# alibaba-mmai-research/CLIP-FSAR

Measured on AMD Instinct MI355X. Metric: episodes/sec (5-way 1-shot, 8 frames, ViT-B/16), higher is better.
Workload: dtype bf16; 1 GPU; BASELINE config[1]: 5-way 1-shot, 1 query/class, 8x224^2 frames, ViT-B/16, random-init CLIP weights, synthetic structured frames; frames_per_episode=80, precision=bf16, parallelism=episodes sharded over 1 rank(s); one all-gather of accuracies, launcher=single process

## Files before the change

### clip-fsar_amd/csrc/gemm_vit.hip

```cpp
#include <type_traits>
#include <utility>

#include "common.h"
#include "gemm_vit.h"

#include "gemm_vit_epi.h"

namespace {

template <typename TI, typename TO, int ACT, int MODE, int OPATH, int STORE, bool SHORTK = false, int MIW = 4>
__global__ __launch_bounds__(512, 2) void vit_gemm_kernel(VitGemmArgs p) {
    static_assert(!SHORTK || OPATH == 1, "K = 128 runs on the LDS-DMA path");
    static_assert(MIW == 4 || (MIW == 3 && !SHORTK), "tile height 256 or 192");
    constexpr int TMv = 64 * MIW;
    constexpr int WR = 32 * MIW;
    constexpr int NM = 2 * MIW;
    constexpr int NL = MIW + 2;
    constexpr bool WIDE = MODE == 6;
    constexpr bool HAS_RES = MODE == 1 || WIDE;
    constexpr bool LNFOLD = MODE == 2 || MODE == 4;
    constexpr bool HB = MODE == 4;
    extern __shared__ __attribute__((aligned(16))) char smem[];
    const int tid = threadIdx.x, lane = tid & 63;
    const int wave = __builtin_amdgcn_readfirstlane(tid >> 6);
// ... 103 lines not shown
    };
    auto tail_pin = [&]() __attribute__((always_inline)) {
        if constexpr (CORR) asm volatile("" : "+v"(tcq[0]), "+v"(tcq[1]));
        if constexpr (LNFOLD)
            asm volatile("" : "+v"(tl[0]), "+v"(tl[1]), "+v"(tl[2]), "+v"(tl[3]), "+v"(tl[4]), "+v"(tl[5]), "+v"(tl[6]), "+v"(tl[7]), "+v"(tl[8]), "+v"(tl[NTL - 1]));
        else
            asm volatile("" : "+v"(tl[0]), "+v"(tl[1]));
    };
    auto tail_fold = [&]() __attribute__((always_inline)) {
        if constexpr (!LNFOLD) {
            typedef typename Vec2B<TI>::v8 TI8;
            TI8 bw[2];
#pragma unroll
            for (int ni = 0; ni < 2; ++ni) {
                const float bv = hi ? 0.f : tl[ni];
                const TI h = (TI)bv;
                const float r1 = bv - (float)h;
                const TI m = (TI)r1;
                const TI l = (TI)(r1 - (float)m);
                TI q = (TI)0.f;
                if constexpr (CORR) q = (TI)tcq[ni];
                bw[ni] = TI8{h, m, l, q, 0, 0, 0, 0};
            }
            const TI one = (TI)(hi ? 0.f : 1.f);
            TI8 ones = TI8{one, one, one, 0, 0, 0, 0, 0};
#pragma unroll
            for (int mi = 0; mi < MIW; ++mi) {
                if constexpr (CORR) {
                    const bool in0 = mi * 32 + lr < corr_bnd;
                    const TI ind = (TI)((p.corr != nullptr && ((in0 ? corr_par : corr_par ^ 1) == hi)) ? 1.f : 0.f);
                    ones = TI8{one, one, one, ind, 0, 0, 0, 0};
                }
#pragma unroll
                for (int ni = 0; ni < 2; ++ni) {
                    if constexpr (std::is_same<TI, _Float16>::value) acc[mi][ni] = __builtin_amdgcn_mfma_f32_32x32x16_f16(bw[ni], ones, acc[mi][ni], 0, 0, 0);
                    else acc[mi][ni] = __builtin_amdgcn_mfma_f32_32x32x16_bf16(bw[ni], ones, acc[mi][ni], 0, 0, 0);
                }
            }
        } else {
            f16x8 cw[2], mx[4];
#pragma unroll
            for (int ni = 0; ni < 2; ++ni) {
                const _Float16 h = (_Float16)tl[ni], l = (_Float16)(tl[ni] - (float)h);
                _Float16 q = (_Float16)0.f;
                if constexpr (CORR) q = (_Float16)tcq[ni];
                cw[ni] = f16x8{h, h, l, q, 0, 0, 0, 0};
            }
#pragma unroll
            for (int mi = 0; mi < MIW; ++mi) {
                const float nm = hi ? tl[2 + mi] : -tl[2 + mi];
                const _Float16 h = (_Float16)nm, l = (_Float16)(nm - (float)h);
                _Float16 sdh = (_Float16)0.f;
                if constexpr (CORR) {
                    const bool in0 = mi * 32 + lr < corr_bnd;
                    sdh = (_Float16)((p.corr != nullptr && ((in0 ? corr_par : corr_par ^ 1) == hi)) ? (p.corr_raw ? 1.0f : __builtin_amdgcn_rcpf(tl[6 + mi])) : 0.f);
                }
                mx[mi] = f16x8{h, l, h, sdh, 0, 0, 0, 0};
                rscale[mi] = tl[6 + mi];
            }
#pragma unroll
            for (int mi = 0; mi < MIW; ++mi)
#pragma unroll
                for (int ni = 0; ni < 2; ++ni)
                    acc[mi][ni] = __builtin_amdgcn_mfma_f32_32x32x16_f16(cw[ni], mx[mi], acc[mi][ni], 0, 0, 0);
        }
    };
    constexpr bool kFuseStats = LNFOLD && OPATH == 2 && MIW == 3;
    const bool fuse_stats = kFuseStats && p.part != nullptr;
    u32x4 sp[4] = {};
    auto stat_loads = [&](auto MI_) __attribute__((always_inline)) {
        constexpr int mi = decltype(MI_)::value;
        int m = m0 + wm * WR + mi * 32 + lr;
        m = m < p.M ? m : p.M - 1;
        const char* src = reinterpret_cast<const char*>(p.part) + ((size_t)m * p.part_slots + (hi ? 8 : 0)) * 8;
        sp[2] = u32x4{0u, 0u, 0u, 0u};
        sp[3] = u32x4{0u, 0u, 0u, 0u};
#ifndef CFSAR_HIDDEN_TAIL_LOADS
        sp[0] = *reinterpret_cast<const u32x4*>(src);
        sp[1] = *reinterpret_cast<const u32x4*>(src + 16);
        if (p.part_slots == 16 || hi == 0) {
            sp[2] = *reinterpret_cast<const u32x4*>(src + 32);
            sp[3] = *reinterpret_cast<const u32x4*>(src + 48);
        }
#else
        asm volatile("global_load_dwordx4 %0, %1, off" : "=v"(sp[0]) : "v"(src) : "memory");
        asm volatile("global_load_dwordx4 %0, %1, off offset:16" : "=v"(sp[1]) : "v"(src) : "memory");
        if (p.part_slots == 16 || hi == 0) {
            asm volatile("global_load_dwordx4 %0, %1, off offset:32" : "+v"(sp[2]) : "v"(src) : "memory");
            asm volatile("global_load_dwordx4 %0, %1, off offset:48" : "+v"(sp[3]) : "v"(src) : "memory");
        }
#endif
    };
    auto stat_consume = [&](auto MI_) __attribute__((always_inline)) {
        constexpr int mi = decltype(MI_)::value;
        asm volatile("" : "+v"(sp[0]), "+v"(sp[1]), "+v"(sp[2]), "+v"(sp[3]));
        auto f = [](unsigned u) { return __builtin_bit_cast(float, u); };
        float s = ((f(sp[0][0]) + f(sp[0][2])) + (f(sp[1][0]) + f(sp[1][2]))) + ((f(sp[2][0]) + f(sp[2][2])) + (f(sp[3][0]) + f(sp[3][2])));
        float sq = ((f(sp[0][1]) + f(sp[0][3])) + (f(sp[1][1]) + f(sp[1][3]))) + ((f(sp[2][1]) + f(sp[2][3])) + (f(sp[3][1]) + f(sp[3][3])));
        const int partner = (lane ^ 32) << 2;
        s += __builtin_bit_cast(float, __builtin_amdgcn_ds_bpermute(partner, __builtin_bit_cast(int, s)));
        sq += __builtin_bit_cast(float, __builtin_amdgcn_ds_bpermute(partner, __builtin_bit_cast(int, sq)));
        const float invD = p.part_invD, eps = p.part_eps;
        const float mean = s * invD;
        const float var = fmaxf(sq * invD - mean * mean, 0.f);
        const float sd = sqrtf(var + eps);
        tl[2 + mi] = hi ? sd : mean;
        tl[6 + mi] = 1.0f / sd;
    };
    auto stats_at = [&](int kstat) __attribute__((always_inline)) {
        if constexpr (kFuseStats) {
            if (fuse_stats && kstat >= 0 && kstat <= MIW) {
                static_for<MIW>([&](auto MI_) {
                    if (kstat == decltype(MI_)::value + 1) stat_consume(MI_);
                });
                static_for<MIW>([&](auto MI_) {
                    if (kstat == decltype(MI_)::value) stat_loads(MI_);
                });
            }
        }
    };
    u32x4 GX[4], GW[4];
    uint4 xfA[4], wfA[2], xfB[4], wfB[2];
    auto gloadX = [&](const unsigned (&ox)[4], int kt, auto J) __attribute__((always_inline)) {
        GX[decltype(J)::value] = *reinterpret_cast<const u32x4*>(p.A + (size_t)(kt >= p.nka ? kt - p.nka : kt) * akstride + ox[decltype(J)::value]);
    };
    auto gloadW = [&](const unsigned (&ow)[4], int kt, auto J) __attribute__((always_inline)) {
        GW[decltype(J)::value] = *reinterpret_cast<const u32x4*>(p.W + (size_t)kt * ROWB + ow[decltype(J)::value]);
    };
    auto swriteX = [&](int stage, auto J) __attribute__((always_inline)) {
        *reinterpret_cast<u32x4*>(smem + stage * STAGE + wr_off + decltype(J)::value * 8192) = GX[decltype(J)::value];
    };
    auto swriteW = [&](int stage, auto J) __attribute__((always_inline)) {
        *reinterpret_cast<u32x4*>(smem + stage * STAGE + TM * ROWB + wr_off + decltype(J)::value * 8192) = GW[decltype(J)::value];
    };
    auto dmaX = [&](const unsigned (&ox)[4], int kt, int stage, auto J) __attribute__((always_inline)) {
        const char* src = p.A + (size_t)(kt >= p.nka ? kt - p.nka : kt) * akstride + ox[decltype(J)::value];
        const unsigned dst = ldsw + (unsigned)stage * (unsigned)STAGE + (unsigned)decltype(J)::value * 8192u;
#ifdef CFSAR_DEV
        if (p.dbg & 4096) { glds16_asm_pol<1>(src, dst); return; }
        if (p.dbg & 16384) { glds16_asm_pol<2>(src, dst); return; }
#endif
        glds16_asm(src, dst);
    };
    auto dmaW = [&](const unsigned (&ow)[4], int kt, int stage, auto J) __attribute__((always_inline)) {
        const char* src = p.W + (size_t)kt * ROWB + ow[decltype(J)::value];
        const unsigned dst = ldsw + (unsigned)stage * (unsigned)STAGE + (unsigned)(TM * ROWB) + (unsigned)decltype(J)::value * 8192u;
#ifdef CFSAR_DEV
        if (p.dbg & 8192) { glds16_asm_pol<1>(src, dst); return; }
#endif
        glds16_asm(src, dst);
    };
    using T_ = std::true_type;
    using F_ = std::false_type;
    auto load_one = [&](int stage, int ss, auto J, uint4 (&xf)[4], uint4 (&wf)[2]) __attribute__((always_inline)) {
        constexpr int j = decltype(J)::value;
        const char* base = smem + stage * STAGE;
        const int x2 = ss << 5;
        constexpr int isx[6] = {1, 0, 1, 1, MIW == 4 ? 1 : 0, 0};
        constexpr int idx[6] = {0, 0, 1, 2, MIW == 4 ? 3 : 1, 1};
        if constexpr (isx[j] != 0) xf[idx[j]] = *reinterpret_cast<const uint4*>(base + (rdX[idx[j]] ^ x2));
        else wf[idx[j]] = *reinterpret_cast<const uint4*>(base + (rdW[idx[j]] ^ x2));
    };
    auto mfma_one = [&](auto J, uint4 (&xf)[4], uint4 (&wf)[2], auto ZERO) __attribute__((always_inline)) {
        constexpr int j = decltype(J)::value;
        constexpr int ni = j / MIW, mi = j % MIW;
        const f32x16 zero = {0.f, 0.f, 0.f, 0.f, 0.f, 0.f, 0.f, 0.f, 0.f, 0.f, 0.f, 0.f, 0.f, 0.f, 0.f, 0.f};
        const f32x16 c = decltype(ZERO)::value ? zero : acc[mi][ni];
        if constexpr (std::is_same<TI, _Float16>::value)
            acc[mi][ni] = __builtin_amdgcn_mfma_f32_32x32x16_f16(__builtin_bit_cast(f16x8, wf[ni]), __builtin_bit_cast(f16x8, xf[mi]), c, 0, 0, 0);
        else
            acc[mi][ni] = __builtin_amdgcn_mfma_f32_32x32x16_bf16(__builtin_bit_cast(bf16x8, wf[ni]), __builtin_bit_cast(bf16x8, xf[mi]), c, 0, 0, 0);
    };
    auto step = [&](int cur, int nxt, const unsigned (&ox)[4], const unsigned (&ow)[4], int ksrc, auto LOAD, auto WRITE, auto SYNC, auto FRAGS, auto ZERO, auto TAIL, int kstat = -1) __attribute__((always_inline)) {
        constexpr bool load = decltype(LOAD)::value, write = decltype(WRITE)::value, sync = decltype(SYNC)::value,
                       frags = decltype(FRAGS)::value, tail = decltype(TAIL)::value;
        static_for<NM>([&](auto J) {
            constexpr int j = decltype(J)::value;
            mfma_one(J, xfA, wfA, ZERO);
            if constexpr (j < NL) load_one(cur, 1, J, xfB, wfB);
            if constexpr (j >= NM - MIW) {
                if constexpr (OPATH == 0) { if constexpr (write) swriteX(nxt, std::integral_constant<int, j - (NM - MIW)>{}); }
                else if constexpr (OPATH == 1) { if constexpr (load) dmaX(ox, ksrc, nxt, std::integral_constant<int, j - (NM - MIW)>{}); }
            }
            __builtin_amdgcn_sched_barrier(0);
        });
        static_for<NM>([&](auto J) {
            constexpr int j = decltype(J)::value;
            mfma_one(J, xfB, wfB, F_{});
            if constexpr (j < NL) load_one(cur, 2, J, xfA, wfA);
            if constexpr (OPATH == 0) {
                if constexpr (j >= NM - MIW && load) gloadX(ox, ksrc, std::integral_constant<int, j - (NM - MIW)>{});
            } else if constexpr (OPATH == 1) {
                if constexpr (j >= NM - 4 && load) dmaW(ow, ksrc, nxt, std::integral_constant<int, j - (NM - 4)>{});
            }
            __builtin_amdgcn_sched_barrier(0);
        });
        static_for<NM>([&](auto J) {
            constexpr int j = decltype(J)::value;
            mfma_one(J, xfA, wfA, F_{});
            if constexpr (j < NL) load_one(cur, 3, J, xfB, wfB);
            if constexpr (j >= NM - 4 && OPATH == 0 && write) swriteW(nxt, std::integral_constant<int, j - (NM - 4)>{});
            __builtin_amdgcn_sched_barrier(0);
        });
        static_for<NM>([&](auto J) {
            constexpr int j = decltype(J)::value;
            mfma_one(J, xfB, wfB, F_{});
            if constexpr (j < 2) {
                if constexpr (OPATH == 0 && load) {
                    gloadW(ow, ksrc, std::integral_constant<int, 2 * j>{});
                    gloadW(ow, ksrc, std::integral_constant<int, 2 * j + 1>{});
                }
            } else if constexpr (frags) {
                load_one(nxt, 0, std::integral_constant<int, j - 2>{}, xfA, wfA);
                if constexpr (j == NM - 1 && NL > NM - 2) load_one(nxt, 0, std::integral_constant<int, NL - 1>{}, xfA, wfA);
            }
            if constexpr (tail && j == 2) tail_loads(m0, n0);
            if constexpr (kFuseStats && j == 2) stats_at(kstat);
            if constexpr (OPATH == 2 && load && j >= 2 && MIW == 4) {
                if constexpr (j < 6) dmaX(ox, ksrc, cur, std::integral_constant<int, j - 2>{});
                else {
                    dmaW(ow, ksrc, cur, std::integral_constant<int, 2 * (j - 6)>{});
                    dmaW(ow, ksrc, cur, std::integral_constant<int, 2 * (j - 6) + 1>{});
                }
            }
            if constexpr (OPATH == 2 && load && j >= 2 && MIW == 3) {
                if constexpr (j == 2) { dmaX(ox, ksrc, cur, std::integral_constant<int, 0>{}); dmaX(ox, ksrc, cur, std::integral_constant<int, 1>{}); }
                if constexpr (j == 3) { dmaX(ox, ksrc, cur, std::integral_constant<int, 2>{}); dmaW(ow, ksrc, cur, std::integral_constant<int, 0>{}); }
                if constexpr (j == 4) { dmaW(ow, ksrc, cur, std::integral_constant<int, 1>{}); dmaW(ow, ksrc, cur, std::integral_constant<int, 2>{}); }
                if constexpr (j == 5) { dmaW(ow, ksrc, cur, std::integral_constant<int, 3>{}); }
            }
            __builtin_amdgcn_sched_barrier(0);
            if constexpr (j == 1 && sync) {
                if constexpr (OPATH >= 1) asm volatile("s_waitcnt vmcnt(0)" ::: "memory");
#ifndef CFSAR_HIDDEN_TAIL_LOADS
                if constexpr (!frags && OPATH >= 1) tail_pin();
#endif
                __syncthreads();
                __builtin_amdgcn_sched_barrier(0);
            }
        });
    };
    origin(b, m0, n0);
    unsigned offX[4], offW[4];
    offsets(m0, n0, offX, offW);
    if constexpr (OPATH == 0) {
        static_for<MIW>([&](auto J) { gloadX(offX, 0, J); });
        static_for<4>([&](auto J) { gloadW(offW, 0, J); });
        static_for<MIW>([&](auto J) { swriteX(0, J); });
        static_for<4>([&](auto J) { swriteW(0, J); });
        static_for<MIW>([&](auto J) { gloadX(offX, 1, J); });
        static_for<4>([&](auto J) { gloadW(offW, 1, J); });
    } else {
        static_for<MIW>([&](auto J) { dmaX(offX, 0, 0, J); });
        static_for<4>([&](auto J) { dmaW(offW, 0, 0, J); });
        if constexpr (OPATH == 2) {
            static_for<MIW>([&](auto J) { dmaX(offX, 1, 1, J); });
            static_for<4>([&](auto J) { dmaW(offW, 1, 1, J); });
            asm volatile("s_waitcnt vmcnt(%0)" : : "n"(MIW + 4) : "memory");
        } else {
            asm volatile("s_waitcnt vmcnt(0)" ::: "memory");
        }
    }
    __syncthreads();
#ifdef CFSAR_DEV
    if (p.dbg & 32768) {
        if (wave >= 4) __builtin_amdgcn_s_setprio(1);
    }
    if (p.dbg & 65536) {
        if (wave < 4) __builtin_amdgcn_s_setprio(1);
    }
#endif
    int sb = 0;
    char* slab = smem + EPI_OFF + wave * EPI_SLAB;
#ifdef CFSAR_DEV
    int trace_i = 0;
    if (p.dbg & 128) {
        const int n = ((blockIdx.x >> 3) & 31) * p.stagger_unit;
        for (int i = 0; i < n; ++i) __builtin_amdgcn_s_sleep(1);
        __syncthreads();
    }
#define CFSAR_TRACE(slot) do { if (p.trace && tid == 0 && trace_i < 64) p.trace[((size_t)blockIdx.x * 64 + trace_i) * 4 + (slot)] = (long long)__builtin_amdgcn_s_memrealtime(); } while (0)
#else
#define CFSAR_TRACE(slot) do { } while (0)
#endif
    for (;;) {
        const int bn = b + grid;
        const bool has_next = bn < nt;
        int m0n = m0, n0n = n0;
        if (has_next) origin(bn, m0n, n0n);
        static_for<NL>([&](auto J) { load_one(sb, 0, J, xfA, wfA); });
        CFSAR_TRACE(0);
        int kt = 0;
        u32x4 rv0[4] = {};
        auto residual_prefetch = [&]() __attribute__((always_inline)) {
            if constexpr (HAS_RES && !WIDE && OPATH >= 1) {
                const int mb_ = m0 + wm * WR, nb_ = n0 + wn * 64;
                const int ncl_ = nb_ + 64 <= p.N ? nb_ : p.N - 64;
                const int rr_ = lane >> 3, Q_ = lane & 7;
#pragma unroll
                for (int it = 0; it < 4; ++it) {
                    int row = mb_ + rr_ + it * 8;
                    row = row < p.M ? row : p.M - 1;
                    rv0[it] = *reinterpret_cast<const u32x4*>(reinterpret_cast<const char*>(p.res) + ((size_t)row * p.ldr + ncl_ + 8 * Q_) * 2);
                }
            }
        };
        if constexpr (OPATH == 0) {
            step(sb & 1, (sb + 1) & 1, offX, offW, 2, T_{}, T_{}, T_{}, T_{}, T_{}, F_{});
            for (kt = 1; kt < nk - 2; ++kt) step((sb + kt) & 1, (sb + kt + 1) & 1, offX, offW, kt + 2, T_{}, T_{}, T_{}, T_{}, F_{}, F_{});
            offsets(m0n, n0n, offX, offW);
            step((sb + kt) & 1, (sb + kt + 1) & 1, offX, offW, 0, T_{}, T_{}, T_{}, T_{}, F_{}, T_{});
            ++kt;
            step((sb + kt) & 1, (sb + kt + 1) & 1, offX, offW, 1, T_{}, T_{}, T_{}, F_{}, F_{}, F_{});
            asm volatile("s_waitcnt vmcnt(%0)" : : "n"(MIW + 4) : "memory");
        } else if constexpr (OPATH == 1 && SHORTK) {
            step(sb & 1, (sb + 1) & 1, offX, offW, 1, T_{}, F_{}, T_{}, T_{}, T_{}, T_{});
            kt = 1;
            offsets(m0n, n0n, offX, offW);
            residual_prefetch();
            step((sb + kt) & 1, (sb + kt + 1) & 1, offX, offW, 0, T_{}, F_{}, T_{}, F_{}, F_{}, F_{});
        } else if constexpr (OPATH == 1) {
            step(sb & 1, (sb + 1) & 1, offX, offW, 1, T_{}, F_{}, T_{}, T_{}, T_{}, F_{});
            for (kt = 1; kt < nk - 2; ++kt) step((sb + kt) & 1, (sb + kt + 1) & 1, offX, offW, kt + 1, T_{}, F_{}, T_{}, T_{}, F_{}, F_{});
            step((sb + kt) & 1, (sb + kt + 1) & 1, offX, offW, kt + 1, T_{}, F_{}, T_{}, T_{}, F_{}, T_{});
            ++kt;
            offsets(m0n, n0n, offX, offW);
            residual_prefetch();
            step((sb + kt) & 1, (sb + kt + 1) & 1, offX, offW, 0, T_{}, F_{}, T_{}, F_{}, F_{}, F_{});
        } else {
            step(sb & 1, (sb + 1) & 1, offX, offW, 2, T_{}, F_{}, T_{}, T_{}, T_{}, F_{}, 0);
            for (kt = 1; kt < nk - 2; ++kt) step((sb + kt) & 1, (sb + kt + 1) & 1, offX, offW, kt + 2, T_{}, F_{}, T_{}, T_{}, F_{}, F_{}, kt);
            offsets(m0n, n0n, offX, offW);
            step((sb + kt) & 1, (sb + kt + 1) & 1, offX, offW, 0, T_{}, F_{}, T_{}, T_{}, F_{}, T_{});
            ++kt;
            residual_prefetch();
            step((sb + kt) & 1, (sb + kt + 1) & 1, offX, offW, 1, T_{}, F_{}, T_{}, F_{}, F_{}, F_{});
        }
        tail_pin();
        tail_fold();
        CFSAR_TRACE(1);
#ifdef CFSAR_DEV
        if (p.dbg & 4) {
            if (acc[0][0][0] == 123.456f) reinterpret_cast<float*>(p.out)[0] = acc[1][1][3] + acc[MIW - 1][1][2] + acc[2][0][1];
        } else
#endif
        {
            const int mb = m0 + wm * WR, nb = n0 + wn * 64;
            if constexpr (WIDE) {
                if (mb + WR <= p.M && nb + 64 <= p.N) epilogue_rows_wide<STORE, true, MIW>(acc, p, mb, nb, lane, slab);
                else epilogue_rows_wide<STORE, false, MIW>(acc, p, mb, nb, lane, slab);
            } else
            if (mb + WR <= p.M && nb + 64 <= p.N) epilogue_rows<TO, ACT, HAS_RES, STORE, true, LNFOLD, HAS_RES && OPATH >= 1, HB, MIW>(acc, p, mb, nb, lane, slab, rscale, rv0);
            else epilogue_rows<TO, ACT, HAS_RES, STORE, false, LNFOLD, HAS_RES && OPATH >= 1, HB, MIW>(acc, p, mb, nb, lane, slab, rscale, rv0);
        }
        CFSAR_TRACE(2);
#ifdef CFSAR_DEV
        ++trace_i;
#endif
        if (!has_next) {
            if constexpr (OPATH == 2) asm volatile("s_waitcnt vmcnt(0)" ::: "memory");
            break;
        }
        sb = (sb + nk) & 1;
        b = bn;
        m0 = m0n;
        n0 = n0n;
    }
}

int persistent_grid() {
    const int n = cfsar_num_cus() & ~7;
    return n >= 8 ? n : 8;
}

constexpr bool vit_has_192(int mode, int opath) {
    return mode == 1 || mode == 6 || ((mode == 2 || mode == 4) && opath == 2);
}

int vit_pick_miw(int M, int tiles_n, int mode, int opath, int K, int dbg) {
    if (K == 128 || !vit_has_192(mode, opath)) return 4;
    const long long G = persistent_grid();
    const long long t256 = (long long)((M + 255) / 256) * tiles_n, t192 = (long long)((M + 191) / 192) * tiles_n;
    const long long r256 = ((t256 + G - 1) / G) * 256, r192 = ((t192 + G - 1) / G) * 192;
    int miw = r192 * 10 <= r256 * 9 ? 3 : 4;
#ifdef CFSAR_DEV
    if (dbg & (1 << 17)) miw = 3;
    if (dbg & (1 << 18)) miw = 4;
#endif
    (void)dbg;
    return miw;
}

template <typename TI, typename TO, int ACT, int MODE, int OPATH, int STORE, bool SHORTK, int MIW = 4>
int launch_inst2(const VitGemmArgs& a, hipStream_t s) {
    auto* fn = &vit_gemm_kernel<TI, TO, ACT, MODE, OPATH, STORE, SHORTK, MIW>;
    if (int rc = cfsar_ensure_lds(reinterpret_cast<const void*>(fn), LDS_BYTES, "cfsar_gemm(vit)")) return rc;
    const int grid = a.ntiles < persistent_grid() ? ((a.ntiles + 7) & ~7) : persistent_grid();
    hipLaunchKernelGGL(fn, dim3(grid), dim3(512), LDS_BYTES, s, a);
    return cfsar_check_launch("cfsar_gemm(vit)");
}

template <typename TI, typename TO, int ACT, int MODE, int OPATH, int STORE>
int launch_inst(const VitGemmArgs& a, hipStream_t s) {
    if (a.K == 128) return launch_inst2<TI, TO, ACT, MODE, 1, STORE, true>(a, s);
    if constexpr (vit_has_192(MODE, OPATH)) {
        if (a.miw == 3) return launch_inst2<TI, TO, ACT, MODE, OPATH, STORE, false, 3>(a, s);
    }
    return launch_inst2<TI, TO, ACT, MODE, OPATH, STORE, false>(a, s);
}

template <int OPATH, int STORE>
int launch_path(const VitGemmArgs& a, int mode, bool f16io, hipStream_t s) {
    if constexpr (STORE == 0) {
        if (mode == 5) return launch_inst<__bf16, __bf16, CFSAR_ACT_NONE, 1, OPATH, STORE>(a, s);
        if (mode == 6) return launch_inst<_Float16, _Float16, CFSAR_ACT_NONE, 6, OPATH, STORE>(a, s);
        if (mode == 1) {
            if (f16io) return launch_inst<_Float16, _Float16, CFSAR_ACT_NONE, 1, OPATH, STORE>(a, s);
            return launch_inst<__bf16, _Float16, CFSAR_ACT_NONE, 1, OPATH, STORE>(a, s);
        }
    } else {
        if (mode == 2) {
            if (f16io) {
                if (a.hb_tokens > 0) return -2;
                if (a.act == CFSAR_ACT_QUICKGELU) return launch_inst<_Float16, _Float16, CFSAR_ACT_QUICKGELU, 2, OPATH, STORE>(a, s);
                return launch_inst<_Float16, _Float16, CFSAR_ACT_NONE, 2, OPATH, STORE>(a, s);
            }
            if (a.act == CFSAR_ACT_QUICKGELU) return launch_inst<_Float16, __bf16, CFSAR_ACT_QUICKGELU, 2, OPATH, STORE>(a, s);
            if (a.hb_tokens > 0) return launch_inst<_Float16, __bf16, CFSAR_ACT_NONE, 4, OPATH, STORE>(a, s);
            return launch_inst<_Float16, __bf16, CFSAR_ACT_NONE, 2, OPATH, STORE>(a, s);
        }
        if (mode == 0) {
            if (a.act == CFSAR_ACT_QUICKGELU) return launch_inst<__bf16, __bf16, CFSAR_ACT_QUICKGELU, 0, OPATH, STORE>(a, s);
            if (a.relu) return launch_inst<__bf16, __bf16, kActRelu, 0, OPATH, STORE>(a, s);
            return launch_inst<__bf16, __bf16, CFSAR_ACT_NONE, 0, OPATH, STORE>(a, s);
        }
    }
    return cfsar_fail("cfsar_gemm (vit): internal: no instance of mode %d with store policy %d", mode, STORE);
}

}

#ifdef CFSAR_DEV
static int g_stagger_unit = 0;
static long long* g_trace = nullptr;
#endif
int cfsar_gemm_vit_try(const VitGemmCall& c, hipStream_t s) {
    const bool lnfold = c.rowstats != nullptr || c.part != nullptr;
    const bool f16io = lnfold ? c.out_dtype == CFSAR_F16 : c.in_dtype == CFSAR_F16;
    const bool f16res = !lnfold && c.out_dtype == CFSAR_F16 && c.res && c.res_dtype == CFSAR_F16 && c.act == CFSAR_ACT_NONE;
    const bool bf16plain = (c.out_dtype == CFSAR_BF16 || (lnfold && c.out_dtype == CFSAR_F16)) && !c.res &&
                           (c.act == CFSAR_ACT_NONE || c.act == CFSAR_ACT_QUICKGELU);
    const bool bf16res = !lnfold && c.in_dtype == CFSAR_BF16 && c.out_dtype == CFSAR_BF16 && c.res && c.res_dtype == CFSAR_BF16 &&
                         c.act == CFSAR_ACT_NONE && c.res != c.out;
    if (!lnfold && c.in_dtype == CFSAR_F16 && !f16res) return -2;
    const bool plainrelu = bf16plain && !lnfold && c.relu && c.act == CFSAR_ACT_NONE && c.out_dtype == CFSAR_BF16 && c.N >= 256;
    if (!(f16res || bf16plain || bf16res) || !c.bias || (c.relu && !(bf16res || plainrelu))) return -2;
    if (lnfold && (!bf16plain || !c.cvec)) return -2;
    if (c.stats_out && !f16res) return -2;
    if (c.K % 64 != 0 || c.K < 128 || c.N % 64 != 0 || c.ldo % 8 != 0 || (c.res && c.ldr % 8 != 0)) return -2;
    if ((size_t)c.M * c.lda * 2 >= (1ull << 32) || (size_t)c.N * c.ldw * 2 >= (1ull << 32) ||
        (size_t)c.M * c.ldo * 2 >= (1ull << 32)) return -2;
    VitGemmArgs a;
    a.A = static_cast<const char*>(c.A);
    a.W = static_cast<const char*>(c.W);
    a.out = c.out;
    a.bias = c.bias;
    a.res = c.res;
    a.rowstats = c.rowstats;
    const int ka = c.ka > 0 ? c.ka : c.K;
    if (!(ka == c.K || (((2 * ka == c.K && ka % 64 == 0) || (3 * ka == 2 * c.K && c.wide && ka % 128 == 0)) && ka >= 128 && c.ha_tokens == 0 &&
                        c.hb_tokens == 0 && c.in_dtype == CFSAR_F16)))
        return cfsar_fail("cfsar_gemm (vit): split operands need K = 2 ka (ka %% 64 == 0) or 2 K = 3 ka (ka %% 128 == 0), fp16 operands, row-major layouts (K=%d, ka=%d)", c.K, ka);
    if (c.wide && !(f16res && c.in_dtype == CFSAR_F16 && c.res == c.out && c.ldr == c.ldo && c.ha_tokens == 0))
        return cfsar_fail("cfsar_gemm_residual_wide: fp16 operands, the residual stream updated in place");
    a.nka = ka / 64;
    a.res_lo = c.wide ? c.res_lo : nullptr;
    a.corr = c.corr;
    a.corr_tokens = c.corr_tokens;
    a.corr_raw = c.corr_raw;
    a.colsum = c.colsum;
    if (c.colsum && !(lnfold && c.act == CFSAR_ACT_QUICKGELU && c.out_dtype == CFSAR_F16 && c.corr_tokens >= 128 && c.hb_tokens == 0))
        return cfsar_fail("cfsar_gemm_lnfold_hp: per-frame output means exist for the fp16 QuickGELU form with >= 128 tokens per frame");
    if (c.corr && !(c.corr_tokens >= 128 && c.in_dtype == CFSAR_F16 && c.out_dtype == CFSAR_F16 && (lnfold || c.wide) && c.hb_tokens == 0))
        return cfsar_fail("cfsar_gemm (vit): the per-frame correction needs >= 128 tokens per frame and an fp16-mode instance (tokens=%d)", c.corr_tokens);
    a.part = c.part; a.part_slots = c.part_slots; a.part_invD = 1.0f / (float)ka; a.part_eps = c.part_eps;
    if (c.part && !(c.pol.opath == 2 && ka >= 512 && (c.part_slots == 12 || c.part_slots == 16) && c.part_slots * 64 == ka))
        return cfsar_fail("cfsar_gemm_lnfold_partials: needs K = 64 slots in {768, 1024} (K=%d, slots=%d)", ka, c.part_slots);
    a.cvec = c.cvec;
    a.stats_out = c.stats_out;
    a.stats_slots = c.N / 64;
    a.M = c.M; a.N = c.N; a.K = c.K;
    a.lda = c.lda; a.ldw = c.ldw; a.ldo = c.ldo; a.ldr = c.ldr;
    a.act = c.act;
    a.relu = c.relu;
    a.tiles_n = (c.N + TN - 1) / TN;
    a.miw = vit_pick_miw(c.M, a.tiles_n, lnfold ? 2 : ((f16res || bf16res) ? (c.wide ? 6 : 1) : 0), c.pol.opath, c.K, c.dbg);
    if (c.part && a.miw != 3) return cfsar_fail("cfsar_gemm_lnfold_partials: internal: fused statistics need the 192-row instance");
    if (c.out_miw) *c.out_miw = a.miw;
    a.ntiles = ((c.M + 64 * a.miw - 1) / (64 * a.miw)) * a.tiles_n;
    a.group = c.pol.group;
    a.colfast = c.pol.colfast;
    a.hb_tokens = c.hb_tokens; a.hb_heads = c.hb_heads; a.ha_tokens = c.ha_tokens;
    if (a.hb_tokens > 0 && !(lnfold && c.act == CFSAR_ACT_NONE && a.hb_tokens >= 128 && a.hb_heads > 0 && c.N == 3 * 64 * a.hb_heads &&
// ... 218 lines not shown
```

### clip-fsar_amd/csrc/gemm_vit_epi.h

```cpp
#pragma once
#include <type_traits>
#include <utility>

#include "common.h"
#include "gemm_vit.h"

namespace {

typedef unsigned u32x4 __attribute__((ext_vector_type(4)));
typedef unsigned u32x2 __attribute__((ext_vector_type(2)));

template <typename F, int... Is>
__device__ __forceinline__ void static_for_impl(F&& f, std::integer_sequence<int, Is...>) {
    (f(std::integral_constant<int, Is>{}), ...);
}
template <int N, typename F>
__device__ __forceinline__ void static_for(F&& f) {
    static_for_impl(static_cast<F&&>(f), std::make_integer_sequence<int, N>{});
}

constexpr int kActRelu = 100;
constexpr int TM = 256, TN = 256;
constexpr int ROWB = 128;
constexpr int STAGE = (TM + TN) * ROWB;
constexpr int EPI_OFF = 2 * STAGE;
constexpr int EPI_SLAB = 32 * 128;
constexpr int LDS_BYTES = EPI_OFF + 8 * EPI_SLAB;

__device__ __forceinline__ int swz(int row) { return (row >> 1) & 7; }

__device__ __forceinline__ void glds16_asm(const char* src, unsigned lds_addr) {
    unsigned keep;
    asm volatile(
        "s_mov_b32 %0, m0\n\t"
        "s_mov_b32 m0, %2\n\t"
        "s_nop 0\n\t"
        "global_load_lds_dwordx4 %1, off\n\t"
        "s_mov_b32 m0, %0"
        : "=&s"(keep)
        : "v"(src), "s"(lds_addr)
        : "memory");
}

#ifdef CFSAR_DEV
template <int POL>
__device__ __forceinline__ void glds16_asm_pol(const char* src, unsigned lds_addr) {
    unsigned keep;
    if constexpr (POL == 1)
        asm volatile("s_mov_b32 %0, m0\n\ts_mov_b32 m0, %2\n\ts_nop 0\n\tglobal_load_lds_dwordx4 %1, off nt\n\ts_mov_b32 m0, %0" : "=&s"(keep) : "v"(src), "s"(lds_addr) : "memory");
    else
        asm volatile("s_mov_b32 %0, m0\n\ts_mov_b32 m0, %2\n\ts_nop 0\n\tglobal_load_lds_dwordx4 %1, off sc1\n\ts_mov_b32 m0, %0" : "=&s"(keep) : "v"(src), "s"(lds_addr) : "memory");
}
#endif

__device__ __forceinline__ void quick_gelu4(float (&v)[4]) {
#pragma unroll
    for (int j = 0; j < 4; ++j) {
        const float z = -1.702f * 1.4426950408889634f * v[j];
        v[j] = v[j] * __builtin_amdgcn_rcpf(1.0f + __builtin_amdgcn_exp2f(z));
    }
}

template <int CTRL>
__device__ __forceinline__ float dpp_move(float v) {
    return __builtin_bit_cast(float, __builtin_amdgcn_update_dpp(0, __builtin_bit_cast(int, v), CTRL, 0xF, 0xF, false));
}
__device__ __forceinline__ float dpp_sum8(float v) {
    v += dpp_move<0xB1>(v);
    v += dpp_move<0x4E>(v);
    v += dpp_move<0x141>(v);
    return v;
}

template <int POLICY>
__device__ __forceinline__ void store16(void* dst, u32x4 v) {
    if constexpr (POLICY == 2) {
        asm volatile("global_store_dwordx4 %0, %1, off sc1 nt\n\ts_nop 1" : : "v"(dst), "v"(v) : "memory");
    } else {
        *reinterpret_cast<u32x4*>(dst) = v;
    }
}

__device__ __forceinline__ void tile_of(int lin, int tiles_m, int tiles_n, int group, int colfast, int& tm, int& tn) {
    const int per = group * tiles_n;
    const int gid = lin / per, first = gid * group;
    const int gsz = tiles_m - first < group ? tiles_m - first : group;
    const int rem = lin - gid * per;
    if (colfast) {
        tm = first + rem / tiles_n;
        tn = rem - (rem / tiles_n) * tiles_n;
    } else {
        tm = first + rem % gsz;
        tn = rem / gsz;
    }
}

template <int HALF>
__device__ __forceinline__ float half_plus(unsigned pair, float c) {
    float r;
    if constexpr (HALF == 0) asm("v_fma_mix_f32 %0, %1, 1.0, %2 op_sel_hi:[1,0,0]" : "=v"(r) : "v"(pair), "v"(c));
    else asm("v_fma_mix_f32 %0, %1, 1.0, %2 op_sel:[1,0,0] op_sel_hi:[1,0,0]" : "=v"(r) : "v"(pair), "v"(c));
    return r;
}

template <typename TO, int ACT, bool HAS_RES, int STORE, bool FULL, bool ROWSCALE = false, bool PRE = false, bool HB = false, int NMI = 4, int CH = 1024>
__device__ __forceinline__ void epilogue_rows(f32x16 (&acc)[NMI][2], const VitGemmArgs& p, int mb, int nb, int lane, char* slab,
                                              const float (&rscale)[4], const u32x4 (&rv0)[4]) {
    typedef typename Vec2B<TO>::v4 TO4;
    typedef typename Vec2B<TO>::v8 TO8;
    const int lr = lane & 31, hi = lane >> 5;
    const int rr = lane >> 3, Q = lane & 7;
    constexpr bool COLSUM = std::is_same<TO, _Float16>::value && ACT == CFSAR_ACT_QUICKGELU && ROWSCALE && !HAS_RES && !HB;
    typedef _Float16 cs_h8 __attribute__((ext_vector_type(8)));
    unsigned cs0[8] = {0, 0, 0, 0, 0, 0, 0, 0}, cs1[8] = {0, 0, 0, 0, 0, 0, 0, 0};
    int cs_bnd = 0, cs_jb = 0, cs_jb0 = 0;
    if constexpr (COLSUM) {
        if (p.colsum != nullptr) {
            cs_bnd = (mb / p.corr_tokens + 1) * p.corr_tokens - mb;
            const int jb = (cs_bnd - rr + 7) >> 3;
            cs_jb = jb < 4 * NMI ? jb : 4 * NMI;
            cs_jb0 = __builtin_amdgcn_readfirstlane(cs_bnd >> 3);
        }
    }
    const bool colok = FULL || nb + 64 <= p.N;
    const int ncl = colok ? nb : p.N - 64;
    char* wr = CH == 1024 ? slab + lr * 128 : slab + (lr >> 3) * CH + (lr & 7) * 128;
    const int wsw = lr & 15;
    const bool swap_halves = rr & 1;
    const unsigned ostep = (unsigned)p.ldo * 16u, rstep = (unsigned)p.ldr * 16u;
    char* outp = reinterpret_cast<char*>(p.out) + ((size_t)(mb + rr) * p.ldo + ncl + 8 * Q) * 2;
    const char* resp = HAS_RES ? reinterpret_cast<const char*>(p.res) + ((size_t)(mb + rr) * p.ldr + ncl + 8 * Q) * 2 : nullptr;
    const int rd0 = rr * 128 + ((Q ^ ((rr >> 1) & 7)) << 4);
    char* hb_base = nullptr;
    size_t hb_wrap = 0;
    int hb_wrap_step = 16;
    if constexpr (HB) {
        const int row0 = mb + rr;
        const int f0 = row0 / p.hb_tokens, t0 = row0 - f0 * p.hb_tokens;
        const int blk = ncl >> 6, which = blk / p.hb_heads, h = blk - which * p.hb_heads;
        const size_t frame_bytes = (size_t)p.hb_heads * p.hb_tokens * 384;
        hb_base = reinterpret_cast<char*>(p.out) + (size_t)f0 * frame_bytes + ((size_t)h * p.hb_tokens + t0) * 384 + which * 128 + Q * 16;
        hb_wrap = frame_bytes - (size_t)p.hb_tokens * 384;
        hb_wrap_step = (p.hb_tokens - t0 + 7) >> 3;
    }
    auto out_addr = [&](int step) __attribute__((always_inline)) -> char* {
        if constexpr (HB) return hb_base + step * 3072 + (step >= hb_wrap_step ? hb_wrap : (size_t)0);
        else return outp + (size_t)step * ostep;
    };
    u32x4 rvn[4];
    auto load_res = [&](int mi_) __attribute__((always_inline)) {
        if constexpr (HAS_RES) {
#pragma unroll
            for (int it = 0; it < 4; ++it) {
                const int step = mi_ * 4 + it;
                if (FULL || mb + rr + step * 8 < p.M) rvn[it] = *reinterpret_cast<const u32x4*>(resp + (size_t)step * rstep);
                else rvn[it] = u32x4{0, 0, 0, 0};
            }
        }
    };
    if constexpr (PRE) {
#pragma unroll
        for (int it = 0; it < 4; ++it) rvn[it] = rv0[it];
    } else {
        load_res(0);
    }
    auto gelu_consts = [&](int mi, float& gk, float& gsd) __attribute__((always_inline)) {
        if constexpr (ROWSCALE && ACT == CFSAR_ACT_QUICKGELU) {
            float rs = rscale[mi];
            asm volatile("" : "+v"(rs));
            gk = -1.702f * 1.4426950408889634f * rs;
            gsd = __builtin_amdgcn_rcpf(rs);
        }
    };
    auto convert_group = [&](int mi, int q, float gk, float gsd) __attribute__((always_inline)) {
        const int ni = q >> 2, g = q & 3;
        TO4 o;
        float v[4];
        if constexpr (ROWSCALE && ACT == CFSAR_ACT_QUICKGELU) {
#pragma unroll
            for (int j = 0; j < 4; ++j) {
                const float a = acc[mi][ni][4 * g + j];
                const float e = __builtin_amdgcn_exp2f(a * gk);
                v[j] = a * __builtin_amdgcn_rcpf(__builtin_fmaf(e, gsd, gsd));
            }
        } else {
#pragma unroll
            for (int j = 0; j < 4; ++j) {
                v[j] = acc[mi][ni][4 * g + j];
                if constexpr (ROWSCALE) v[j] *= rscale[mi];
            }
            if constexpr (ACT == CFSAR_ACT_QUICKGELU) quick_gelu4(v);
            if constexpr (ACT == kActRelu) {
#pragma unroll
                for (int j = 0; j < 4; ++j) v[j] = fmaxf(v[j], 0.0f);
            }
        }
#pragma unroll
        for (int j = 0; j < 4; ++j) o[j] = (TO)v[j];
        const int slot = (2 * (ni * 4 + g) + hi) ^ wsw;
        *reinterpret_cast<TO4*>(wr + slot * 8) = o;
    };
    auto read_back = [&](u32x4 (&d)[4]) __attribute__((always_inline)) {
#pragma unroll
        for (int it = 0; it < 4; ++it)
            d[it] = *reinterpret_cast<const u32x4*>(slab + it * CH + (rd0 ^ ((it & 1) << 6)));
    };
    auto finish = [&](int mi, int it, u32x4 x, u32x4 r) __attribute__((always_inline)) {
        const bool rowok = FULL || mb + rr + (mi * 4 + it) * 8 < p.M;
        if (swap_halves) x = u32x4{x[2], x[3], x[0], x[1]};
        if constexpr (HAS_RES && std::is_same<TO, _Float16>::value) {
            typedef _Float16 h2 __attribute__((ext_vector_type(2)));
            const h2 ones = {(_Float16)1.0f, (_Float16)1.0f};
            float ps = 0.f, pq = 0.f;
            const TO8 s8 = __builtin_bit_cast(TO8, x) + __builtin_bit_cast(TO8, r);
            x = __builtin_bit_cast(u32x4, s8);
            if (p.stats_out) {
                const h2 s01 = __builtin_shufflevector(s8, s8, 0, 1), s23 = __builtin_shufflevector(s8, s8, 2, 3);
                const h2 s45 = __builtin_shufflevector(s8, s8, 4, 5), s67 = __builtin_shufflevector(s8, s8, 6, 7);
                ps = __builtin_amdgcn_fdot2(s01, ones, ps, false);
                pq = __builtin_amdgcn_fdot2(s01, s01, pq, false);
                ps = __builtin_amdgcn_fdot2(s23, ones, ps, false);
                pq = __builtin_amdgcn_fdot2(s23, s23, pq, false);
                ps = __builtin_amdgcn_fdot2(s45, ones, ps, false);
                pq = __builtin_amdgcn_fdot2(s45, s45, pq, false);
                ps = __builtin_amdgcn_fdot2(s67, ones, ps, false);
                pq = __builtin_amdgcn_fdot2(s67, s67, pq, false);
                ps = dpp_sum8(ps);
                pq = dpp_sum8(pq);
                if (Q == 0 && (FULL || (rowok && colok)))
                    *reinterpret_cast<float2*>(p.stats_out + ((size_t)(mb + rr + (mi * 4 + it) * 8) * p.stats_slots + (nb >> 6)) * 2) =
                        make_float2(ps, pq);
            }
        } else if constexpr (HAS_RES) {
            const TO8 a = __builtin_bit_cast(TO8, x), b = __builtin_bit_cast(TO8, r);
            TO8 sres;
#pragma unroll
            for (int j = 0; j < 8; ++j) {
                float t = (float)a[j] + (float)b[j];
                if (p.relu) t = fmaxf(t, 0.0f);
                sres[j] = (TO)t;
            }
            x = __builtin_bit_cast(u32x4, sres);
        }
#ifdef CFSAR_DEV
        if ((p.dbg & 16) && x[0] != 0x7fc12345u) return;
        if ((p.dbg & 32) && ((blockIdx.x >> 3) & 1) && x[0] != 0x7fc12345u) return;
#endif
        if (FULL || (rowok && colok)) store16<STORE>(out_addr(mi * 4 + it), x);
        if constexpr (COLSUM) {
            if (p.colsum != nullptr) {
                typedef _Float16 cs_h2 __attribute__((ext_vector_type(2)));
                const int j_ = mi * 4 + it;
                if (j_ == cs_jb0 || j_ == cs_jb0 + 1) {
#pragma unroll
                    for (int e = 0; e < 8; ++e) cs0[e] = (j_ == cs_jb) ? cs1[e] : cs0[e];
                }
                constexpr float kMagic = 1.5f * 2048.0f;
                const cs_h2 lim = {(_Float16)1000.0f, (_Float16)1000.0f};
#pragma unroll
                for (int k = 0; k < 4; ++k) {
                    const unsigned xw = x[k];
                    cs_h2 hv = __builtin_bit_cast(cs_h2, xw);
                    hv = __builtin_elementwise_min(__builtin_elementwise_max(hv, -lim), lim);
                    const unsigned cw = __builtin_bit_cast(unsigned, hv);
                    const unsigned b0 = __builtin_bit_cast(unsigned, half_plus<0>(cw, kMagic)), b1 = __builtin_bit_cast(unsigned, half_plus<1>(cw, kMagic));
                    cs1[2 * k] += (FULL || rowok) ? b0 : __builtin_bit_cast(unsigned, kMagic);
                    cs1[2 * k + 1] += (FULL || rowok) ? b1 : __builtin_bit_cast(unsigned, kMagic);
                }
            }
        }
    };
#pragma unroll
    for (int mi = 0; mi < NMI; ++mi) {
        u32x4 rv[4];
#pragma unroll
        for (int it = 0; it < 4; ++it) {
            if constexpr (HAS_RES) rv[it] = rvn[it];
        }
        if (mi < NMI - 1) load_res(mi + 1);
        float gk = 0.f, gsd = 0.f;
        gelu_consts(mi, gk, gsd);
#pragma unroll
        for (int q = 0; q < 8; ++q) convert_group(mi, q, gk, gsd);
        u32x4 d[4];
        read_back(d);
#pragma unroll
        for (int it = 0; it < 4; ++it) finish(mi, it, d[it], rv[it]);
    }
    if constexpr (COLSUM) {
        if (p.colsum != nullptr) {
            const int partner = (lane ^ 32) << 2;
            constexpr unsigned kbits = 0x45400000u;
            static_assert(__builtin_bit_cast(unsigned, 1.5f * 2048.0f) == kbits, "magic constant");
#pragma unroll
            for (int j = 0; j < 8; ++j) {
                int a0 = (int)((cs_jb >= 4 * NMI ? cs1[j] : cs0[j]) - (unsigned)cs_jb * kbits);
                int a1 = (int)(cs1[j] - (unsigned)(4 * NMI) * kbits) - a0;
                a0 += __builtin_amdgcn_update_dpp(0, a0, 0x128, 0xF, 0xF, false);
                a1 += __builtin_amdgcn_update_dpp(0, a1, 0x128, 0xF, 0xF, false);
                a0 += __builtin_amdgcn_ds_swizzle(a0, 0x401F);
                a1 += __builtin_amdgcn_ds_swizzle(a1, 0x401F);
                a0 += __builtin_amdgcn_ds_bpermute(partner, a0);
                a1 += __builtin_amdgcn_ds_bpermute(partner, a1);
                cs0[j] = (unsigned)a0;
                cs1[j] = (unsigned)a1;
            }
            if (rr == 0 && colok && mb < p.M) {
                int* dst = reinterpret_cast<int*>(p.colsum) + ((size_t)(mb / (32 * NMI)) * 2) * p.N + ncl + 8 * Q;
                *reinterpret_cast<u32x4*>(dst) = u32x4{cs0[0], cs0[1], cs0[2], cs0[3]};
                *reinterpret_cast<u32x4*>(dst + 4) = u32x4{cs0[4], cs0[5], cs0[6], cs0[7]};
                *reinterpret_cast<u32x4*>(dst + p.N) = u32x4{cs1[0], cs1[1], cs1[2], cs1[3]};
                *reinterpret_cast<u32x4*>(dst + p.N + 4) = u32x4{cs1[4], cs1[5], cs1[6], cs1[7]};
            }
        }
    }
}

template <int HALF>
__device__ __forceinline__ float mix_sum(unsigned a, unsigned b) {
    float r;
    if constexpr (HALF == 0) asm("v_fma_mix_f32 %0, %1, 1.0, %2 op_sel_hi:[1,0,1]" : "=v"(r) : "v"(a), "v"(b));
    else asm("v_fma_mix_f32 %0, %1, 1.0, %2 op_sel:[1,0,1] op_sel_hi:[1,0,1]" : "=v"(r) : "v"(a), "v"(b));
    return r;
}
template <int HALF>
__device__ __forceinline__ float mix_sub(unsigned pair, float c) {
    float r;
    if constexpr (HALF == 0) asm("v_fma_mix_f32 %0, %1, -1.0, %2 op_sel_hi:[1,0,0]" : "=v"(r) : "v"(pair), "v"(c));
    else asm("v_fma_mix_f32 %0, %1, -1.0, %2 op_sel:[1,0,0] op_sel_hi:[1,0,0]" : "=v"(r) : "v"(pair), "v"(c));
    return r;
}

template <int STORE, bool FULL, int NMI, int CH = 1024>
__device__ __forceinline__ void epilogue_rows_wide(f32x16 (&acc)[NMI][2], const VitGemmArgs& p, int mb, int nb, int lane, char* slab) {
    typedef _Float16 h2 __attribute__((ext_vector_type(2)));
    typedef _Float16 h8 __attribute__((ext_vector_type(8)));
    typedef float f4 __attribute__((ext_vector_type(4)));
    const int lr = lane & 31, hi = lane >> 5;
    const int rr = lane >> 2, Q = lane & 3;
    const bool colok = FULL || nb + 64 <= p.N;
    const int ncl = colok ? nb : p.N - 64;
    const int wsw = ((lr >> 1) & 7) ^ ((lr & 1) << 2);
    const int rsw = ((rr >> 1) & 7) ^ ((rr & 1) << 2);
    char* wr = CH == 1024 ? slab + lr * 128 : slab + (lr >> 3) * CH + (lr & 7) * 128;
    const char* rd = CH == 1024 ? slab + rr * 128 : slab + (rr >> 3) * CH + (rr & 7) * 128;
    const bool has_lo = p.res_lo != nullptr;
    const size_t eoff = ((size_t)(mb + rr) * p.ldo + ncl + 8 * Q) * 2;
    char* outp = reinterpret_cast<char*>(p.out) + eoff;
    char* lop = has_lo ? reinterpret_cast<char*>(p.res_lo) + eoff : nullptr;
    const unsigned rstep = (unsigned)p.ldo * 32u;
    u32x4 rh[2], rl[2], nh[2], nl[2];
    auto load_res = [&](int pass) __attribute__((always_inline)) {
        const int mi_ = pass >> 1, ni_ = pass & 1;
#pragma unroll
        for (int it = 0; it < 2; ++it) {
            const int step = mi_ * 2 + it;
            const bool ok = FULL || mb + rr + step * 16 < p.M;
            const size_t o = (size_t)step * rstep + ni_ * 64;
            nh[it] = ok ? *reinterpret_cast<const u32x4*>(outp + o) : u32x4{0, 0, 0, 0};
            nl[it] = (ok && has_lo) ? *reinterpret_cast<const u32x4*>(lop + o) : u32x4{0, 0, 0, 0};
        }
    };
    load_res(0);
    float ps[2] = {0.f, 0.f}, pq[2] = {0.f, 0.f};
#pragma unroll
    for (int pass = 0; pass < 2 * NMI; ++pass) {
        const int mi = pass >> 1, ni = pass & 1;
#pragma unroll
        for (int it = 0; it < 2; ++it) { rh[it] = nh[it]; rl[it] = nl[it]; }
        if (pass + 1 < 2 * NMI) load_res(pass + 1);
#pragma unroll
        for (int g = 0; g < 4; ++g) {
            const f4 v = {acc[mi][ni][4 * g], acc[mi][ni][4 * g + 1], acc[mi][ni][4 * g + 2], acc[mi][ni][4 * g + 3]};
            *reinterpret_cast<f4*>(wr + (((2 * g + hi) ^ wsw) << 4)) = v;
        }
#pragma unroll
        for (int it = 0; it < 2; ++it) {
            const f4 a = *reinterpret_cast<const f4*>(rd + it * 2 * CH + (((2 * Q) ^ rsw) << 4));
            const f4 b = *reinterpret_cast<const f4*>(rd + it * 2 * CH + (((2 * Q + 1) ^ rsw) << 4));
            u32x4 ohw, olw;
#pragma unroll
            for (int k = 0; k < 4; ++k) {
                const float d0 = k < 2 ? a[2 * k] : b[2 * k - 4], d1 = k < 2 ? a[2 * k + 1] : b[2 * k - 3];
                const float s0 = d0 + mix_sum<0>(rh[it][k], rl[it][k]);
                const float s1 = d1 + mix_sum<1>(rh[it][k], rl[it][k]);
                const h2 hp = {(_Float16)s0, (_Float16)s1};
                const unsigned hb = __builtin_bit_cast(unsigned, hp);
                const h2 lp = {(_Float16)mix_sub<0>(hb, s0), (_Float16)mix_sub<1>(hb, s1)};
                ohw[k] = hb;
                olw[k] = __builtin_bit_cast(unsigned, lp);
            }
            const h8 oh = __builtin_bit_cast(h8, ohw), ol = __builtin_bit_cast(h8, olw);
            const int step = mi * 2 + it;
            const bool rowok = FULL || mb + rr + step * 16 < p.M;
            if (p.stats_out) {
                const h2 ones = {(_Float16)1.0f, (_Float16)1.0f};
                const h2 s01 = __builtin_shufflevector(oh, oh, 0, 1), s23 = __builtin_shufflevector(oh, oh, 2, 3);
                const h2 s45 = __builtin_shufflevector(oh, oh, 4, 5), s67 = __builtin_shufflevector(oh, oh, 6, 7);
                float s_ = 0.f, q_ = 0.f;
                s_ = __builtin_amdgcn_fdot2(s01, ones, s_, false);
                q_ = __builtin_amdgcn_fdot2(s01, s01, q_, false);
                s_ = __builtin_amdgcn_fdot2(s23, ones, s_, false);
                q_ = __builtin_amdgcn_fdot2(s23, s23, q_, false);
                s_ = __builtin_amdgcn_fdot2(s45, ones, s_, false);
                q_ = __builtin_amdgcn_fdot2(s45, s45, q_, false);
                s_ = __builtin_amdgcn_fdot2(s67, ones, s_, false);
                q_ = __builtin_amdgcn_fdot2(s67, s67, q_, false);
                s_ += dpp_move<0xB1>(s_);
                q_ += dpp_move<0xB1>(q_);
                s_ += dpp_move<0x4E>(s_);
                q_ += dpp_move<0x4E>(q_);
                if (ni == 0) { ps[it] = s_; pq[it] = q_; }
                else {
                    ps[it] += s_; pq[it] += q_;
                    if (Q == 0 && (FULL || (rowok && colok)))
                        *reinterpret_cast<float2*>(p.stats_out + ((size_t)(mb + rr + step * 16) * p.stats_slots + (nb >> 6)) * 2) =
                            make_float2(ps[it], pq[it]);
                }
            }
            if (FULL || (rowok && colok)) {
                const size_t o = (size_t)step * rstep + ni * 64;
                store16<STORE>(outp + o, __builtin_bit_cast(u32x4, oh));
                if (has_lo) store16<STORE>(lop + o, __builtin_bit_cast(u32x4, ol));
            }
        }
    }
}

}
```

Before: 347.4 episodes/s.

## Overlap next tile's first k-step MFMAs with LN-fold GEMM epilogue

```diff
diff --git a/clip-fsar_amd/csrc/gemm_vit.hip b/clip-fsar_amd/csrc/gemm_vit.hip
--- a/clip-fsar_amd/csrc/gemm_vit.hip
+++ b/clip-fsar_amd/csrc/gemm_vit.hip
@@ -279,20 +279,23 @@
     };
     using T_ = std::true_type;
     using F_ = std::false_type;
-    auto load_one = [&](int stage, int ss, auto J, uint4 (&xf)[4], uint4 (&wf)[2]) __attribute__((always_inline)) {
+    auto load_one = [&](int stage, int ss, auto J, uint4 (&xf)[4], uint4 (&wf)[2], auto ONLY_LAST) __attribute__((always_inline)) {
         constexpr int j = decltype(J)::value;
         const char* base = smem + stage * STAGE;
         const int x2 = ss << 5;
         constexpr int isx[6] = {1, 0, 1, 1, MIW == 4 ? 1 : 0, 0};
         constexpr int idx[6] = {0, 0, 1, 2, MIW == 4 ? 3 : 1, 1};
-        if constexpr (isx[j] != 0) xf[idx[j]] = *reinterpret_cast<const uint4*>(base + (rdX[idx[j]] ^ x2));
-        else wf[idx[j]] = *reinterpret_cast<const uint4*>(base + (rdW[idx[j]] ^ x2));
+        if constexpr (isx[j] != 0) {
+            if constexpr (!decltype(ONLY_LAST)::value || idx[j] == MIW - 1) xf[idx[j]] = *reinterpret_cast<const uint4*>(base + (rdX[idx[j]] ^ x2));
+        } else wf[idx[j]] = *reinterpret_cast<const uint4*>(base + (rdW[idx[j]] ^ x2));
     };
     auto mfma_one = [&](auto J, uint4 (&xf)[4], uint4 (&wf)[2], auto ZERO) __attribute__((always_inline)) {
         constexpr int j = decltype(J)::value;
         constexpr int ni = j / MIW, mi = j % MIW;
+        constexpr int zmode = (int)decltype(ZERO)::value;
+        if constexpr ((zmode & 2) != 0 && mi != MIW - 1) return;
         const f32x16 zero = {0.f, 0.f, 0.f, 0.f, 0.f, 0.f, 0.f, 0.f, 0.f, 0.f, 0.f, 0.f, 0.f, 0.f, 0.f, 0.f};
-        const f32x16 c = decltype(ZERO)::value ? zero : acc[mi][ni];
+        const f32x16 c = (zmode & 1) ? zero : acc[mi][ni];
         if constexpr (std::is_same<TI, _Float16>::value)
             acc[mi][ni] = __builtin_amdgcn_mfma_f32_32x32x16_f16(__builtin_bit_cast(f16x8, wf[ni]), __builtin_bit_cast(f16x8, xf[mi]), c, 0, 0, 0);
         else
@@ -301,10 +304,12 @@
     auto step = [&](int cur, int nxt, const unsigned (&ox)[4], const unsigned (&ow)[4], int ksrc, auto LOAD, auto WRITE, auto SYNC, auto FRAGS, auto ZERO, auto TAIL, int kstat = -1) __attribute__((always_inline)) {
         constexpr bool load = decltype(LOAD)::value, write = decltype(WRITE)::value, sync = decltype(SYNC)::value,
                        frags = decltype(FRAGS)::value, tail = decltype(TAIL)::value;
+        using REST_ = std::integral_constant<int, (int)decltype(ZERO)::value & 2>;
+        using OL_ = std::integral_constant<bool, ((int)decltype(ZERO)::value & 2) != 0>;
         static_for<NM>([&](auto J) {
             constexpr int j = decltype(J)::value;
             mfma_one(J, xfA, wfA, ZERO);
-            if constexpr (j < NL) load_one(cur, 1, J, xfB, wfB);
+            if constexpr (j < NL) load_one(cur, 1, J, xfB, wfB, OL_{});
             if constexpr (j >= NM - MIW) {
                 if constexpr (OPATH == 0) { if constexpr (write) swriteX(nxt, std::integral_constant<int, j - (NM - MIW)>{}); }
                 else if constexpr (OPATH == 1) { if constexpr (load) dmaX(ox, ksrc, nxt, std::integral_constant<int, j - (NM - MIW)>{}); }
@@ -313,8 +318,8 @@
         });
         static_for<NM>([&](auto J) {
             constexpr int j = decltype(J)::value;
-            mfma_one(J, xfB, wfB, F_{});
-            if constexpr (j < NL) load_one(cur, 2, J, xfA, wfA);
+            mfma_one(J, xfB, wfB, REST_{});
+            if constexpr (j < NL) load_one(cur, 2, J, xfA, wfA, OL_{});
             if constexpr (OPATH == 0) {
                 if constexpr (j >= NM - MIW && load) gloadX(ox, ksrc, std::integral_constant<int, j - (NM - MIW)>{});
             } else if constexpr (OPATH == 1) {
@@ -324,22 +329,22 @@
         });
         static_for<NM>([&](auto J) {
             constexpr int j = decltype(J)::value;
-            mfma_one(J, xfA, wfA, F_{});
-            if constexpr (j < NL) load_one(cur, 3, J, xfB, wfB);
+            mfma_one(J, xfA, wfA, REST_{});
+            if constexpr (j < NL) load_one(cur, 3, J, xfB, wfB, OL_{});
             if constexpr (j >= NM - 4 && OPATH == 0 && write) swriteW(nxt, std::integral_constant<int, j - (NM - 4)>{});
             __builtin_amdgcn_sched_barrier(0);
         });
         static_for<NM>([&](auto J) {
             constexpr int j = decltype(J)::value;
-            mfma_one(J, xfB, wfB, F_{});
+            mfma_one(J, xfB, wfB, REST_{});
             if constexpr (j < 2) {
                 if constexpr (OPATH == 0 && load) {
                     gloadW(ow, ksrc, std::integral_constant<int, 2 * j>{});
                     gloadW(ow, ksrc, std::integral_constant<int, 2 * j + 1>{});
                 }
             } else if constexpr (frags) {
-                load_one(nxt, 0, std::integral_constant<int, j - 2>{}, xfA, wfA);
-                if constexpr (j == NM - 1 && NL > NM - 2) load_one(nxt, 0, std::integral_constant<int, NL - 1>{}, xfA, wfA);
+                load_one(nxt, 0, std::integral_constant<int, j - 2>{}, xfA, wfA, F_{});
+                if constexpr (j == NM - 1 && NL > NM - 2) load_one(nxt, 0, std::integral_constant<int, NL - 1>{}, xfA, wfA, F_{});
             }
             if constexpr (tail && j == 2) tail_loads(m0, n0);
             if constexpr (kFuseStats && j == 2) stats_at(kstat);
@@ -366,6 +371,32 @@
                 __builtin_amdgcn_sched_barrier(0);
             }
         });
+    };
+    constexpr bool OVL = LNFOLD && OPATH == 2;
+#ifdef CFSAR_DEV
+    const bool ovl = OVL && !(p.dbg & (1 << 23));
+#else
+    constexpr bool ovl = OVL;
+#endif
+    int ostage = 0;
+    uint4 ofx[2], ofw[2][2];
+    auto ovl_block = [&](int mi, int q) __attribute__((always_inline)) {
+        const char* base = smem + ostage * STAGE;
+        auto rd = [&](int ss) __attribute__((always_inline)) {
+            const int x2 = ss << 5;
+            ofx[ss & 1] = *reinterpret_cast<const uint4*>(base + (rdX[mi] ^ x2));
+            ofw[ss & 1][0] = *reinterpret_cast<const uint4*>(base + (rdW[0] ^ x2));
+            ofw[ss & 1][1] = *reinterpret_cast<const uint4*>(base + (rdW[1] ^ x2));
+        };
+        if (q < 0) { rd(0); return; }
+        const int ss = q >> 1, ni = q & 1;
+        if (ni == 0 && ss < 3) rd(ss + 1);
+        const f32x16 zero = {0.f, 0.f, 0.f, 0.f, 0.f, 0.f, 0.f, 0.f, 0.f, 0.f, 0.f, 0.f, 0.f, 0.f, 0.f, 0.f};
+        const f32x16 c = ss == 0 ? zero : acc[mi][ni];
+        if constexpr (std::is_same<TI, _Float16>::value)
+            acc[mi][ni] = __builtin_amdgcn_mfma_f32_32x32x16_f16(__builtin_bit_cast(f16x8, ofw[ss & 1][ni]), __builtin_bit_cast(f16x8, ofx[ss & 1]), c, 0, 0, 0);
+        else
+            acc[mi][ni] = __builtin_amdgcn_mfma_f32_32x32x16_bf16(__builtin_bit_cast(bf16x8, ofw[ss & 1][ni]), __builtin_bit_cast(bf16x8, ofx[ss & 1]), c, 0, 0, 0);
     };
     origin(b, m0, n0);
     unsigned offX[4], offW[4];
@@ -397,6 +428,14 @@
         if (wave < 4) __builtin_amdgcn_s_setprio(1);
     }
 #endif
+    if constexpr (OVL) {
+        if (ovl) {
+#pragma unroll
+            for (int mi = 0; mi < MIW - 1; ++mi)
+#pragma unroll
+                for (int q = -1; q < 8; ++q) ovl_block(mi, q);
+        }
+    }
     int sb = 0;
     char* slab = smem + EPI_OFF + wave * EPI_SLAB;
 #ifdef CFSAR_DEV
@@ -415,7 +454,7 @@
         const bool has_next = bn < nt;
         int m0n = m0, n0n = n0;
         if (has_next) origin(bn, m0n, n0n);
-        static_for<NL>([&](auto J) { load_one(sb, 0, J, xfA, wfA); });
+        static_for<NL>([&](auto J) { load_one(sb, 0, J, xfA, wfA, F_{}); });
         CFSAR_TRACE(0);
         int kt = 0;
         u32x4 rv0[4] = {};
@@ -455,7 +494,11 @@
             residual_prefetch();
             step((sb + kt) & 1, (sb + kt + 1) & 1, offX, offW, 0, T_{}, F_{}, T_{}, F_{}, F_{}, F_{});
         } else {
-            step(sb & 1, (sb + 1) & 1, offX, offW, 2, T_{}, F_{}, T_{}, T_{}, T_{}, F_{}, 0);
+            bool masked = false;
+            if constexpr (OVL) {
+                if (ovl) { step(sb & 1, (sb + 1) & 1, offX, offW, 2, T_{}, F_{}, T_{}, T_{}, std::integral_constant<int, 3>{}, F_{}, 0); masked = true; }
+            }
+            if (!masked) step(sb & 1, (sb + 1) & 1, offX, offW, 2, T_{}, F_{}, T_{}, T_{}, T_{}, F_{}, 0);
             for (kt = 1; kt < nk - 2; ++kt) step((sb + kt) & 1, (sb + kt + 1) & 1, offX, offW, kt + 2, T_{}, F_{}, T_{}, T_{}, F_{}, F_{}, kt);
             offsets(m0n, n0n, offX, offW);
             step((sb + kt) & 1, (sb + kt + 1) & 1, offX, offW, 0, T_{}, F_{}, T_{}, T_{}, F_{}, T_{});
@@ -476,6 +519,12 @@
             if constexpr (WIDE) {
                 if (mb + WR <= p.M && nb + 64 <= p.N) epilogue_rows_wide<STORE, true, MIW>(acc, p, mb, nb, lane, slab);
                 else epilogue_rows_wide<STORE, false, MIW>(acc, p, mb, nb, lane, slab);
+            } else
+            if (OVL && ovl && has_next) {
+                if constexpr (OVL) {
+                    ostage = (sb + nk) & 1;
+                    epilogue_rows<TO, ACT, HAS_RES, STORE, false, LNFOLD, false, HB, MIW, 1024, true>(acc, p, mb, nb, lane, slab, rscale, rv0, ovl_block);
+                }
             } else
             if (mb + WR <= p.M && nb + 64 <= p.N) epilogue_rows<TO, ACT, HAS_RES, STORE, true, LNFOLD, HAS_RES && OPATH >= 1, HB, MIW>(acc, p, mb, nb, lane, slab, rscale, rv0);
             else epilogue_rows<TO, ACT, HAS_RES, STORE, false, LNFOLD, HAS_RES && OPATH >= 1, HB, MIW>(acc, p, mb, nb, lane, slab, rscale, rv0);
diff --git a/clip-fsar_amd/csrc/gemm_vit_epi.h b/clip-fsar_amd/csrc/gemm_vit_epi.h
--- a/clip-fsar_amd/csrc/gemm_vit_epi.h
+++ b/clip-fsar_amd/csrc/gemm_vit_epi.h
@@ -103,9 +103,10 @@
     return r;
 }
 
-template <typename TO, int ACT, bool HAS_RES, int STORE, bool FULL, bool ROWSCALE = false, bool PRE = false, bool HB = false, int NMI = 4, int CH = 1024>
+template <typename TO, int ACT, bool HAS_RES, int STORE, bool FULL, bool ROWSCALE = false, bool PRE = false, bool HB = false, int NMI = 4, int CH = 1024,
+          bool OVLP = false, typename OV = int>
 __device__ __forceinline__ void epilogue_rows(f32x16 (&acc)[NMI][2], const VitGemmArgs& p, int mb, int nb, int lane, char* slab,
-                                              const float (&rscale)[4], const u32x4 (&rv0)[4]) {
+                                              const float (&rscale)[4], const u32x4 (&rv0)[4], OV&& ovl = OV{}) {
     typedef typename Vec2B<TO>::v4 TO4;
     typedef typename Vec2B<TO>::v8 TO8;
     const int lr = lane & 31, hi = lane >> 5;
@@ -280,8 +281,17 @@
         if (mi < NMI - 1) load_res(mi + 1);
         float gk = 0.f, gsd = 0.f;
         gelu_consts(mi, gk, gsd);
-#pragma unroll
-        for (int q = 0; q < 8; ++q) convert_group(mi, q, gk, gsd);
+        if constexpr (OVLP) {
+            if (mi >= 1) ovl(mi - 1, -1);
+        }
+#pragma unroll
+        for (int q = 0; q < 8; ++q) {
+            if constexpr (OVLP) {
+                if (mi >= 1) ovl(mi - 1, q);
+            }
+            convert_group(mi, q, gk, gsd);
+            if constexpr (OVLP) __builtin_amdgcn_sched_barrier(0);
+        }
         u32x4 d[4];
         read_back(d);
 #pragma unroll
```

Result: no change. 345.8 episodes/s (-0.4%).
